# refresh-bio/agc

Hardware: AMD Instinct MI355X
Metric: input Gbp/s compressed (create), hot path FASTA bytes in HBM -> 2-bit pack + scan + match + encode + zstd packing (higher is better)
Workload: dtype u8

## Files before the change

### agc_amd/capi.py

```python
import ctypes as C
import os

import numpy as np

HERE = os.path.dirname(os.path.abspath(__file__))
LIB_PATH = os.path.join(HERE, "libagc_hip.so")

OK, ENODEV, EINVAL, ENOMEM, ECAP, ENOREF = 0, -1, -2, -3, -4, -5
K_SCAN, K_INDEX, K_ENCODE, K_ESTIMATE, K_COSTVEC, K_REVCOMP, K_PREPROCESS, K_REFSTORE = range(8)
K_NAMES = ["scan", "index", "encode", "estimate", "costvec", "revcomp", "preprocess", "refstore", "zstd", "filter", "segments", "pack"]

SYMBOLS = [
    "agc_hip_create", "agc_hip_destroy", "agc_hip_last_error", "agc_hip_abi_version", "agc_hip_sync",
    "agc_hip_timing_enable", "agc_hip_timing_reset", "agc_hip_timing_get",
    "agc_hip_sample_buffer", "agc_hip_copy_to_device",
    "agc_hip_preprocess_dev", "agc_hip_preprocess",
    "agc_hip_splitters_set", "agc_hip_splitters_insert", "agc_hip_splitters_count",
    "agc_hip_determine_splitters_dev",
    "agc_hip_scan_contigs_dev", "agc_hip_scan_contigs",
    "agc_hip_ref_register", "agc_hip_ref_register_batch_dev", "agc_hip_ref_get", "agc_hip_ref_index_get",
    "agc_hip_lz_encode_batch_dev", "agc_hip_lz_encode_batch", "agc_hip_lz_encode_begin_dev", "agc_hip_lz_encode_end", "agc_hip_lz_encode_pending",
    "agc_hip_lz_encode_begin_packed_on", "agc_hip_lz_encode_end_on", "agc_hip_lz_encode_pending_on", "agc_hip_lz_encode_drop_on",
    "agc_hip_host_alloc", "agc_hip_host_free",
    "agc_hip_lz_estimate_batch_dev", "agc_hip_lz_estimate_batch",
    "agc_hip_lz_cost_vector_batch_dev", "agc_hip_lz_cost_vector_batch",
    "agc_hip_lz_split_point_batch_dev", "agc_hip_fetch_slices_dev",
    "agc_hip_ref_lag_counts_dev",
    "agc_hip_zstd17_max_input", "agc_hip_zstd17_resident_frames", "agc_hip_zstd17_batch", "agc_hip_zstd17_batch_dev", "agc_hip_zstd17_background", "agc_hip_zstd17_cparams", "agc_hip_zstd_batch", "agc_hip_zstd_cparams",
    "agc_hip_packed_words_bytes", "agc_hip_packed_index_bytes", "agc_hip_pack_dev", "agc_hip_expand_dev", "agc_hip_scan_packed_dev",
    "agc_hip_prefetch_packed_dev", "agc_hip_scan_prefetched", "agc_hip_sample_pack", "agc_hip_sample_pack_fasta", "agc_hip_ref_store_begin_packed", "agc_hip_ref_store_end",
    "agc_hip_ref_register_batch_packed", "agc_hip_lz_encode_batch_packed", "agc_hip_lz_encode_begin_packed", "agc_hip_lz_estimate_batch_packed",
    "agc_hip_lz_cost_vector_batch_packed", "agc_hip_lz_split_point_batch_packed", "agc_hip_fetch_slices_packed", "agc_hip_ref_lag_counts_packed",
    "agc_hip_pack_fasta_begin", "agc_hip_pack_fasta_end", "agc_hip_pack_fasta_dev",
    "agc_hip_group_hash", "agc_hip_group_map_set", "agc_hip_group_map_update", "agc_hip_segments_packed", "agc_hip_segments_encode_known",
]

u8p = C.POINTER(C.c_uint8)
u32p = C.POINTER(C.c_uint32)
u64p = C.POINTER(C.c_uint64)
vp = C.c_void_p


class Packed(C.Structure):
    _fields_ = [("d_words", C.c_void_p), ("d_esc_index", C.c_void_p), ("d_esc_bytes", C.c_void_p), ("n_symbols", C.c_uint64)]


class GroupSlot(C.Structure):
    _fields_ = [("k1", C.c_uint64), ("k2", C.c_uint64), ("gid", C.c_int32), ("used", C.c_uint32)]


class Segment(C.Structure):
    _fields_ = [("start", C.c_uint64), ("front_dir", C.c_uint64), ("front_rc", C.c_uint64), ("back_dir", C.c_uint64), ("back_rc", C.c_uint64),
                ("ctg", C.c_uint32), ("len", C.c_uint32), ("map_gid", C.c_int32), ("front_full", C.c_uint8), ("back_full", C.c_uint8),
                ("store_rc", C.c_uint8), ("encoded", C.c_uint8)]


# ... 58 lines not shown
    L.agc_hip_lz_estimate_batch_dev.argtypes = [vp, C.c_uint32, u32p, vp, u64p, u32p, u8p, u32p, u32p]
    L.agc_hip_lz_estimate_batch.argtypes = [vp, C.c_uint32, u32p, u8p, u64p, u32p, u8p, u32p, u32p]
    L.agc_hip_lz_cost_vector_batch_dev.argtypes = [vp, C.c_uint32, u32p, vp, u64p, u32p, u8p, u8p, u32p]
    L.agc_hip_lz_cost_vector_batch.argtypes = [vp, C.c_uint32, u32p, u8p, u64p, u32p, u8p, u8p, u32p]
    L.agc_hip_lz_split_point_batch_dev.argtypes = [vp, C.c_uint32, u32p, u32p, vp, u64p, u32p, u8p, u8p, u8p, u8p, u32p, u32p]
    L.agc_hip_fetch_slices_dev.argtypes = [vp, C.c_uint32, vp, u64p, u32p, u8p, u8p, C.c_uint64, u64p]
    L.agc_hip_ref_lag_counts_dev.argtypes = [vp, C.c_uint32, vp, u64p, u32p, u8p, u32p, u32p]
    L.agc_hip_zstd17_batch.argtypes = [vp, C.c_uint32, u8p, u64p, u8p, C.c_uint64, u64p]
    L.agc_hip_zstd17_cparams.argtypes = [C.c_uint64, u32p]
    L.agc_hip_zstd_cparams.argtypes = [C.c_int, C.c_uint64, u32p]
    L.agc_hip_zstd_batch.argtypes = [vp, C.c_uint32, u8p, u64p, u8p, u8p, C.c_uint64, u64p]
    L.agc_hip_zstd17_batch_dev.argtypes = [vp, C.c_uint32, vp, u64p, u8p, C.c_uint64, u64p]
    L.agc_hip_zstd17_background.argtypes = [vp, C.c_int]
    L.agc_hip_zstd17_max_input.restype = C.c_uint32
    L.agc_hip_zstd17_resident_frames.argtypes = [vp]
    L.agc_hip_zstd17_resident_frames.restype = C.c_uint32
    L.agc_hip_packed_words_bytes.restype = C.c_uint64
    L.agc_hip_packed_words_bytes.argtypes = [C.c_uint64]
    L.agc_hip_packed_index_bytes.restype = C.c_uint64
    L.agc_hip_packed_index_bytes.argtypes = [C.c_uint64]
    L.agc_hip_pack_dev.argtypes = [vp, vp, C.c_uint64, vp, vp, vp, C.c_uint64, u64p]
    L.agc_hip_pack_fasta_begin.argtypes = [vp, vp, C.c_uint64, u64p, u64p, C.c_uint32, vp, vp, vp, C.c_uint64]
    L.agc_hip_pack_fasta_end.argtypes = [vp, u64p, u64p]
    L.agc_hip_pack_fasta_dev.argtypes = [vp, vp, C.c_uint64, u64p, u64p, C.c_uint32, vp, vp, vp, C.c_uint64, u64p, u64p]
    L.agc_hip_expand_dev.argtypes = [vp, C.POINTER(Packed), vp]
    L.agc_hip_scan_packed_dev.argtypes = [vp, C.POINTER(Packed), u64p, C.c_uint32, C.c_uint32, C.c_uint64, u64p, u32p, u64p, u64p, u64p]
    L.agc_hip_prefetch_packed_dev.argtypes = [vp, C.POINTER(Packed), u64p, C.c_uint32, C.c_uint32]
    pkp = C.POINTER(Packed)
    L.agc_hip_sample_pack.argtypes = [vp, vp, C.c_uint64, pkp]
    L.agc_hip_ref_store_begin_packed.argtypes = [vp, C.c_uint32, C.c_uint32, C.c_uint32, pkp, u64p, C.POINTER(C.c_uint32), vp, vp, vp, vp, C.c_uint64, u64p]
    L.agc_hip_ref_store_end.argtypes = [vp, C.c_uint32]
    L.agc_hip_sample_pack_fasta.argtypes = [vp, C.c_uint32, C.POINTER(C.c_char_p), u64p, pkp, u64p]
    L.agc_hip_ref_register_batch_packed.argtypes = [vp, C.c_uint32, u32p, pkp, u64p, u32p, u8p, C.c_uint32]
    L.agc_hip_lz_encode_batch_packed.argtypes = [vp, C.c_uint32, u32p, pkp, u64p, u32p, u8p, u8p, C.c_uint64, u64p]
    L.agc_hip_lz_encode_begin_packed.argtypes = [vp, C.c_uint32, u32p, pkp, u64p, u32p, u8p]
    L.agc_hip_lz_encode_begin_packed_on.argtypes = [vp, C.c_uint32, C.c_uint32, u32p, pkp, u64p, u32p, u8p]
    L.agc_hip_lz_encode_end_on.argtypes = [vp, C.c_uint32, u8p, C.c_uint64, u64p]
    L.agc_hip_lz_encode_pending_on.argtypes = [vp, C.c_uint32, u32p]
    L.agc_hip_lz_encode_drop_on.argtypes = [vp, C.c_uint32]
    L.agc_hip_lz_estimate_batch_packed.argtypes = [vp, C.c_uint32, u32p, pkp, u64p, u32p, u8p, u32p, u32p]
    L.agc_hip_lz_cost_vector_batch_packed.argtypes = [vp, C.c_uint32, u32p, pkp, u64p, u32p, u8p, u8p, u32p]
    L.agc_hip_lz_split_point_batch_packed.argtypes = [vp, C.c_uint32, u32p, u32p, pkp, u64p, u32p, u8p, u8p, u8p, u8p, u32p, u32p]
    L.agc_hip_fetch_slices_packed.argtypes = [vp, C.c_uint32, pkp, u64p, u32p, u8p, u8p, C.c_uint64, u64p]
    L.agc_hip_ref_lag_counts_packed.argtypes = [vp, C.c_uint32, pkp, u64p, u32p, u8p, u32p, u32p]
    L.agc_hip_group_hash.argtypes = [C.c_uint64, C.c_uint64]
    L.agc_hip_group_hash.restype = C.c_uint64
# ... 152 lines not shown
        self._chk(self.L.agc_hip_pack_fasta_begin(self.h, d_raw_tensor.data_ptr(), int(n_raw), _p(rb, u64p), _p(re_, u64p), rb.size, words.data_ptr(),
                                                  index.data_ptr(), esc.data_ptr(), esc_cap))
        return {"raw": d_raw_tensor, "n_raw": int(n_raw), "rb": rb, "re": re_, "bufs": (words, index, esc)}

    def pack_fasta_end(self, pending):
        import torch
        while True:
            off = np.zeros(pending["rb"].size + 1, np.uint64)
            cnt = np.zeros(1, np.uint64)
            rc = self.L.agc_hip_pack_fasta_end(self.h, _p(off, u64p), _p(cnt, u64p))
            if rc == ECAP:
                words, index, _esc = pending["bufs"]
                esc = torch.empty((int(cnt[0]) + 16) * 1024, dtype=torch.uint8, device=words.device)
                torch.cuda.synchronize(words.device)
                pending = self.pack_fasta_begin(pending["raw"], pending["n_raw"], pending["rb"], pending["re"], bufs=(words, index, esc))
                continue
            self._chk(rc)
            words, index, esc = pending["bufs"]
            return Packed(words.data_ptr(), index.data_ptr(), esc.data_ptr(), int(off[-1])), pending["bufs"], off

    def pack_fasta_dev(self, d_raw_tensor, n_raw, raw_begin, raw_end, esc_cap=64):
        return self.pack_fasta_end(self.pack_fasta_begin(d_raw_tensor, n_raw, raw_begin, raw_end, esc_cap))

    def expand_dev(self, pk, d_codes_ptr):
        self._chk(self.L.agc_hip_expand_dev(self.h, C.byref(pk), d_codes_ptr))
        self._chk(self.L.agc_hip_sync(self.h))

    def scan_packed_dev(self, pk, ctg_off, k, cap=1 << 16):
        fn = lambda h, arg, *rest: self.L.agc_hip_scan_packed_dev(h, C.byref(arg), *rest)
        return self._scan(fn, pk, ctg_off, k, cap)

    def prefetch_packed_dev(self, pk, ctg_off, k):
        off = _a(ctg_off, np.uint64)
        self._chk(self.L.agc_hip_prefetch_packed_dev(self.h, C.byref(pk), _p(off, u64p), off.size - 1, k))

    def sample_pack(self, d_codes_ptr, n_symbols):
        pk = Packed()
        self._chk(self.L.agc_hip_sample_pack(self.h, d_codes_ptr, n_symbols, C.byref(pk)))
        return pk

    def sample_pack_fasta(self, bodies):
        n = len(bodies)
        ptr = (C.c_char_p * max(n, 1))(*bodies)
        ln = np.array([len(b) for b in bodies], np.uint64)
        off = np.zeros(n + 1, np.uint64)
        pk = Packed()
# ... 287 lines not shown
```

### agc_amd/csrc/api.hip

```cpp
#include "../../include/agc_hip.h"
#include "dev_common.h"

#include <algorithm>
#include <atomic>
#include <chrono>
#include <cstdio>
#include <cstring>
#include <future>
#include <mutex>
#include <numeric>
#include <string>
#include <vector>

#include "scan_kernels.hip"
#include "pack_kernels.hip"
#include "lz_kernels.hip"
#include "seg_kernels.hip"
#include "zstd_kernels.hip"

using namespace agc;

namespace {

struct DevBuf {
// ... 100 lines not shown
        bool done_valid = false;
        hipStream_t s = nullptr;
    } l2, l3;
    hipStream_t stream2 = nullptr, stream3 = nullptr;
    Lane2 &lane(int which) { return which == 2 ? l3 : l2; }

    struct Prefetch {
        hipStream_t stream = nullptr;
        DevBuf d_ranges, d_hits, d_counter;
        uint32_t *h_count = nullptr;
        const void *words = nullptr;
        uint64_t n_symbols = 0;
        uint32_t dev_cap = 0, k = 0, n_ctg = 0;
        uint64_t first_off = 0, last_off = 0;
        bool valid = false, scanned = false;
        hipEvent_t e0 = nullptr, e1 = nullptr;
        bool timed = false;
    } pf;

    struct PackFasta {
        hipStream_t stream = nullptr;
        DevBuf d_state, d_rng, d_off;
        DevBuf d_tcnt, d_toff;
        uint64_t *h_res = nullptr;
        size_t h_res_cap = 0;
        uint32_t n_ctg = 0;
        uint64_t n_raw = 0, esc_cap = 0;
        bool pending = false, timed = false;
        hipEvent_t e0 = nullptr, e1 = nullptr;
    } pfa;

    struct ChunkBufs {
        DevBuf d_jobs, d_seg0, d_logs, d_logn, d_out;
        std::future<DevBuf> logs_ahead;
        bool logs_asked = false;
    } chunk_bufs[3];

    std::vector<void *> host_allocs;

    bool timing = false;
    hipEvent_t ev0 = nullptr, ev1 = nullptr, zev0 = nullptr, zev1 = nullptr;
    struct TimerPair {
        hipEvent_t a = nullptr, b = nullptr;
        int which = -1;
    };
    std::vector<TimerPair> tpairs;
// ... 885 lines not shown
    uint64_t prev = 0;
    for (uint32_t i = 0; i < n_ctg; ++i) {
        if (h_raw_begin[i] < prev || h_raw_end[i] < h_raw_begin[i] || h_raw_end[i] > n_raw)
            return AGC_HIP_EINVAL;
        prev = h_raw_end[i];
    }
    const uint64_t n_tiles64 = (n_raw + PF_TILE - 1) / PF_TILE;
    if (n_tiles64 > 0x7fffffffULL)
        return AGC_HIP_EINVAL;
    HIPCHK(c, hipSetDevice(c->device));
    agc_hip_ctx::PackFasta &P = c->pfa;
    if (!P.stream) {
        HIPCHK(c, hipStreamCreateWithFlags(&P.stream, hipStreamNonBlocking));
        HIPCHK(c, hipEventCreate(&P.e0));
        HIPCHK(c, hipEventCreate(&P.e1));
    }
    if (P.pending) {
        HIPCHK(c, hipStreamSynchronize(P.stream));
        P.pending = false;
    }
    P.n_ctg = n_ctg;
    P.n_raw = n_raw;
    P.esc_cap = esc_cap_blocks;
    const size_t res_words = (size_t)n_ctg + 4;
    if (P.h_res_cap < res_words) {
        if (P.h_res)
            HIPCHK(c, hipHostFree(P.h_res));
        P.h_res = nullptr;
        P.h_res_cap = 0;
        HIPCHK(c, hipHostMalloc((void **)&P.h_res, (res_words + 1024) * 8, hipHostMallocDefault));
        P.h_res_cap = res_words + 1024;
    }
    const uint32_t n_tiles = (uint32_t)n_tiles64;
    CHK(ensure(c, P.d_state, 64, P.stream));
    CHK(ensure(c, P.d_rng, std::max<size_t>(16, (size_t)n_ctg * 16), P.stream));
    CHK(ensure(c, P.d_off, ((size_t)n_ctg + 2) * 8, P.stream));
    HIPCHK(c, hipMemsetAsync(P.d_state.p, 0, 64, P.stream));
    HIPCHK(c, hipMemsetAsync(P.d_off.p, 0xFF, ((size_t)n_ctg + 1) * 8, P.stream));
    if (n_ctg) {
        CHK(upload(c, P.d_rng.p, h_raw_begin, (size_t)n_ctg * 8, P.stream));
        CHK(upload(c, (uint8_t *)P.d_rng.p + (size_t)n_ctg * 8, h_raw_end, (size_t)n_ctg * 8, P.stream));
    }
    P.timed = c->timing;
    if (P.timed)
        (void)hipEventRecord(P.e0, P.stream);
    if (n_tiles && n_ctg) {
        PackFastaArgs a;
        a.raw = d_raw;
        a.n_raw = n_raw;
        a.rng_begin = (const uint64_t *)P.d_rng.p;
        a.rng_end = a.rng_begin + n_ctg;
        a.n_rng = n_ctg;
        a.n_tiles = n_tiles;
        a.esc_count = (uint32_t *)P.d_state.p + 1;
        a.total = (unsigned long long *)P.d_state.p + 1;
        a.words = d_words;
        a.esc_index = d_esc_index;
        a.esc_bytes = d_esc_bytes;
        a.esc_cap = (uint32_t)std::min<uint64_t>(esc_cap_blocks, 0x7fffffffu);
        a.ctg_off = (unsigned long long *)P.d_off.p;
        {
            const uint32_t n_sb = (n_tiles + PF_SCAN_TILES - 1) / PF_SCAN_TILES;
            const size_t tl_bytes = ((size_t)n_tiles * 4 + 255) & ~(size_t)255;
            CHK(ensure(c, P.d_tcnt, tl_bytes + (size_t)n_sb * 4 + 64, P.stream));
            CHK(ensure(c, P.d_toff, tl_bytes + (size_t)n_sb * 8 + 64, P.stream));
            uint32_t *d_cnt = (uint32_t *)P.d_tcnt.p, *d_tot = (uint32_t *)((uint8_t *)P.d_tcnt.p + tl_bytes);
            uint32_t *d_local = (uint32_t *)P.d_toff.p;
            uint64_t *d_boff = (uint64_t *)((uint8_t *)P.d_toff.p + tl_bytes);
            a.tile_local = d_local;
            a.block_off = d_boff;
            hipLaunchKernelGGL(pack_fasta_count_kernel, dim3(n_tiles), dim3(256), 0, P.stream, a, d_cnt);
            hipLaunchKernelGGL(pack_fasta_scan_kernel, dim3(n_sb), dim3(1024), 0, P.stream, (const uint32_t *)d_cnt, n_tiles, d_local, d_tot);
            hipLaunchKernelGGL(pp_scan_kernel, dim3(1), dim3(1024), 0, P.stream, (const uint32_t *)d_tot, n_sb, d_boff,
                               (uint64_t *)((uint8_t *)P.d_state.p + 32));
            hipLaunchKernelGGL(pack_fasta_kernel, dim3(n_tiles), dim3(256), 0, P.stream, a);
        }
        HIPCHK(c, hipGetLastError());
    }
    if (P.timed)
        (void)hipEventRecord(P.e1, P.stream);
    HIPCHK(c, hipMemcpyAsync(P.h_res, P.d_off.p, ((size_t)n_ctg + 1) * 8, hipMemcpyDeviceToHost, P.stream));
    HIPCHK(c, hipMemcpyAsync(P.h_res + n_ctg + 1, P.d_state.p, 16, hipMemcpyDeviceToHost, P.stream));
    P.pending = true;
    return AGC_HIP_OK;
}

int agc_hip_pack_fasta_end(agc_hip_ctx *c, uint64_t *h_ctg_off, uint64_t *h_n_esc_blocks)
{
    if (!c || !h_ctg_off || !h_n_esc_blocks)
        return AGC_HIP_EINVAL;
    agc_hip_ctx::PackFasta &P = c->pfa;
    if (!P.pending)
        return AGC_HIP_EINVAL;
    HIPCHK(c, hipSetDevice(c->device));
    HIPCHK(c, hipStreamSynchronize(P.stream));
    P.pending = false;
    if (P.timed) {
        float ms = 0;
        (void)hipEventElapsedTime(&ms, P.e0, P.e1);
        c->ms[AGC_HIP_K_PACK] += ms;
        c->launches[AGC_HIP_K_PACK] += 1;
        P.timed = false;
    }
    const uint32_t n = P.n_ctg;
    const uint32_t *cnt = (const uint32_t *)(P.h_res + n + 1);
    const uint64_t total = (P.n_raw && n) ? P.h_res[n + 2] : 0;
    for (uint32_t i = 0; i < n; ++i)
        h_ctg_off[i] = P.h_res[i] == ~0ULL ? total : P.h_res[i];
    h_ctg_off[n] = total;
    *h_n_esc_blocks = (P.n_raw && n) ? cnt[1] : 0;
    return *h_n_esc_blocks > P.esc_cap ? AGC_HIP_ECAP : AGC_HIP_OK;
}

int agc_hip_pack_fasta_dev(agc_hip_ctx *c, const uint8_t *d_raw, uint64_t n_raw, const uint64_t *h_raw_begin, const uint64_t *h_raw_end, uint32_t n_ctg,
                           uint32_t *d_words, int32_t *d_esc_index, uint8_t *d_esc_bytes, uint64_t esc_cap_blocks, uint64_t *h_ctg_off, uint64_t *h_n_esc_blocks)
{
    if (!h_ctg_off || !h_n_esc_blocks)
        return AGC_HIP_EINVAL;
    CHK(agc_hip_pack_fasta_begin(c, d_raw, n_raw, h_raw_begin, h_raw_end, n_ctg, d_words, d_esc_index, d_esc_bytes, esc_cap_blocks));
    return agc_hip_pack_fasta_end(c, h_ctg_off, h_n_esc_blocks);
}

int agc_hip_sample_pack_fasta(agc_hip_ctx *c, uint32_t n_ctg, const uint8_t *const *h_raw, const uint64_t *h_len, agc_hip_packed *out, uint64_t *h_ctg_off)
{
    if (!c || !out || !h_ctg_off || (n_ctg && (!h_raw || !h_len)))
        return AGC_HIP_EINVAL;
    *out = agc_hip_packed{};
    HIPCHK(c, hipSetDevice(c->device));
    if (c->pfa.pending) {
        c->err = "sample_pack_fasta: a conversion queued by agc_hip_pack_fasta_begin is pending";
        return AGC_HIP_EINVAL;
    }
    std::vector<uint64_t> rb(n_ctg), re(n_ctg);
    uint64_t tot = 0;
    for (uint32_t i = 0; i < n_ctg; ++i) {
// ... 1744 lines not shown
```

### agc_amd/csrc/pack_kernels.hip

```cpp
#pragma once

namespace agc {

constexpr uint32_t PF_TILE = 16384;
constexpr uint32_t PF_MAX_BLOCKS = PF_TILE / PACK_BLOCK + 1;

struct PackFastaArgs {
    const uint8_t *raw;
    uint64_t n_raw;
    const uint64_t *rng_begin, *rng_end;
    uint32_t n_rng;
    uint32_t n_tiles;
    const uint32_t *tile_local;
    const uint64_t *block_off;
    uint32_t *words;
    int32_t *esc_index;
    uint8_t *esc_bytes;
    uint32_t *esc_count;
    uint32_t esc_cap;
    unsigned long long *ctg_off;
    unsigned long long *total;
};

struct PfChunk {
    uint32_t bits;
    uint32_t cnt;
    uint32_t keep;
    uint32_t other;
};

__device__ __forceinline__ uint8_t pf_byte(const uint32_t w[4], uint32_t j)
{
    const uint32_t q = j >> 2, x = q == 0 ? w[0] : q == 1 ? w[1] : q == 2 ? w[2] : w[3];
    return (uint8_t)(x >> (8 * (j & 3)));
}

__device__ __forceinline__ uint32_t pf_ge64(uint32_t w) { return ((w << 1) | w) & 0x80808080u; }

__device__ __forceinline__ uint32_t pf_gather16(uint32_t f0, uint32_t f1, uint32_t f2, uint32_t f3)
{
    uint32_t v = (f0 >> 7) | (f1 >> 6) | (f2 >> 5) | (f3 >> 4);
    v = (v | (v >> 4)) & 0x00FF00FFu;
    v = (v | (v >> 8)) & 0xFFFFu;
    uint32_t t = ((v >> 3) ^ v) & 0x0A0Au;
// ... 131 lines not shown
            lds_flag[li / PACK_BLOCK] = 1;
        if (first < 16 && (other >> first))
            lds_flag[li / PACK_BLOCK + 1] = 1;
    }
}

__device__ __forceinline__ void pf_escape(const PackFastaArgs &a, const int32_t *lds_slot, uint64_t g, uint32_t keep, const uint32_t w[4], uint64_t s0, uint64_t s1)
{
    for (uint32_t m = keep; m; m &= m - 1, ++g) {
        if (g < s0 || g >= s1)
            continue;
        const int32_t slot = lds_slot[(g - s0) / PACK_BLOCK];
        if (slot >= 0)
            a.esc_bytes[(uint64_t)slot * PACK_BLOCK + ((g - s0) & (PACK_BLOCK - 1))] = cnv_symbol(pf_byte(w, __builtin_ctz(m)));
    }
}

__global__ void __launch_bounds__(256) pack_fasta_count_kernel(PackFastaArgs a, uint32_t *__restrict__ tile_cnt)
{
    __shared__ uint32_t s_part[4], s_rfirst;
    __shared__ unsigned long long s_cb, s_ce;
    const uint32_t tid = threadIdx.x, lane = tid & 63, wv = tid >> 6, tile = blockIdx.x;
    const uint64_t t_begin = (uint64_t)tile * PF_TILE;
    if (tid == 0) {
        uint32_t lo = 0, hi = a.n_rng;
        while (lo < hi) {
            const uint32_t mid = (lo + hi) >> 1;
            if (a.rng_end[mid] <= t_begin)
                lo = mid + 1;
            else
                hi = mid;
        }
        s_rfirst = lo;
        s_cb = lo < a.n_rng ? a.rng_begin[lo] : ~0ULL;
        s_ce = lo < a.n_rng ? a.rng_end[lo] : 0;
    }
    __syncthreads();
    const uint32_t r_first = s_rfirst;
    const uint64_t cb = s_cb, ce = s_ce;
    uint32_t c = 0;
#pragma unroll
    for (uint32_t j = 0; j < 4; ++j) {
        const uint64_t p = t_begin + (uint64_t)wv * 4096 + j * 1024 + lane * 16;
        if (p >= a.n_raw)
            continue;
        uint32_t w[4] = {0, 0, 0, 0};
// ... 4 lines not shown
#pragma unroll
            for (uint32_t t = 0; t < 16; ++t)
                if (p + t < a.n_raw)
                    w[t >> 2] |= (uint32_t)a.raw[p + t] << (8 * (t & 3));
        }
        const uint32_t m0 = pf_ge64(w[0]), m1 = pf_ge64(w[1]), m2 = pf_ge64(w[2]), m3 = pf_ge64(w[3]);
        if (p >= cb && p + 16 <= ce)
            c += __popc(m0) + __popc(m1) + __popc(m2) + __popc(m3);
        else
            c += __popc(pf_gather16(m0, m1, m2, m3) & pf_range_mask(a, p, cb, ce, r_first));
    }
#pragma unroll
    for (int o = 32; o > 0; o >>= 1)
        c += __shfl_down(c, o);
    if (lane == 0)
        s_part[wv] = c;
    __syncthreads();
    if (tid == 0)
        tile_cnt[tile] = s_part[0] + s_part[1] + s_part[2] + s_part[3];
}

constexpr uint32_t PF_SCAN_TILES = 8192;
__global__ void __launch_bounds__(1024) pack_fasta_scan_kernel(const uint32_t *__restrict__ tile_cnt, uint32_t n_tiles, uint32_t *__restrict__ tile_local,
                                                              uint32_t *__restrict__ block_total)
{
    __shared__ uint32_t s_w[16];
    const uint32_t tid = threadIdx.x, lane = tid & 63, wv = tid >> 6;
    const uint32_t t0 = blockIdx.x * PF_SCAN_TILES + tid * 8;
    uint32_t v[8], sum = 0;
#pragma unroll
    for (uint32_t j = 0; j < 8; ++j) {
        v[j] = t0 + j < n_tiles ? tile_cnt[t0 + j] : 0u;
        sum += v[j];
    }
    const uint32_t incl = pf_wave_incl(sum);
    if (lane == 63)
        s_w[wv] = incl;
    __syncthreads();
    uint32_t base = 0, total = 0;
#pragma unroll
    for (uint32_t x = 0; x < 16; ++x) {
        if (x < wv)
            base += s_w[x];
        total += s_w[x];
    }
    uint32_t run = base + incl - sum;
#pragma unroll
    for (uint32_t j = 0; j < 8; ++j) {
        if (t0 + j < n_tiles)
            tile_local[t0 + j] = run;
        run += v[j];
    }
    if (tid == 0)
        block_total[blockIdx.x] = total;
}

__global__ void __launch_bounds__(256) pack_fasta_kernel(PackFastaArgs a)
{
    __shared__ uint32_t s_words[PF_MAX_BLOCKS * (PACK_BLOCK / 16)];
    __shared__ uint32_t s_flag[PF_MAX_BLOCKS];
    __shared__ int32_t s_slot[PF_MAX_BLOCKS];
    __shared__ uint32_t s_wsum[4 * 4];
    __shared__ uint32_t s_tile, s_rfirst;
    __shared__ unsigned long long s_excl, s_cb, s_ce;
    __shared__ uint32_t s_ra[4];
    const uint32_t tid = threadIdx.x, lane = tid & 63, wv = tid >> 6;

    if (tid == 0)
        s_tile = blockIdx.x;
    for (uint32_t i = tid; i < PF_MAX_BLOCKS * (PACK_BLOCK / 16); i += 256)
        s_words[i] = 0;
    if (tid < PF_MAX_BLOCKS) {
        s_flag[tid] = 0;
        s_slot[tid] = -1;
    }
    __syncthreads();
    const uint32_t tile = s_tile;
    if (tile >= a.n_tiles)
        return;
    const uint64_t t_begin = (uint64_t)tile * PF_TILE, t_end = t_begin + PF_TILE < a.n_raw ? t_begin + PF_TILE : a.n_raw;
    if (tid == 0) {
        uint32_t lo = 0, hi = a.n_rng;
        while (lo < hi) {
            const uint32_t mid = (lo + hi) >> 1;
            if (a.rng_end[mid] <= t_begin)
                lo = mid + 1;
            else
                hi = mid;
        }
        s_rfirst = lo;
// ... 109 lines not shown
    p_next = t_begin + PF_TILE;
    for (uint32_t r = 0; r < n_rounds; ++r) {
        uint32_t wr[4];
        const uint32_t need = (uint32_t)(s1 - g_next), span = min(4096u, (need + need / 16 + 47) & ~15u);
        const PfChunk c = pf_chunk(a, tid * 16 < span ? p_next + tid * 16 : a.n_raw, cb, ce, r_first, wr);
        const uint32_t incl = pf_wave_incl(c.cnt);
        __syncthreads();
        if (lane == 63)
            s_ra[wv] = incl;
        __syncthreads();
        uint32_t base = 0, tot = 0;
#pragma unroll
        for (uint32_t x = 0; x < 4; ++x) {
            if (x < wv)
                base += s_ra[x];
            tot += s_ra[x];
        }
        pf_escape(a, s_slot, g_next + base + incl - c.cnt, c.keep, wr, s0, s1);
        g_next += tot;
        p_next += span;
    }
}

}
```

### agc_amd/csrc/scan_kernels.hip

```cpp
#include "dev_common.h"

namespace agc {

__device__ __forceinline__ uint32_t pack4(uint32_t w)
{
    return ((w & 0x03030303u) * 0x40100401u) >> 24;
}

__device__ __forceinline__ uint32_t inv4(uint32_t w)
{
    uint32_t v = w & 0xFCFCFCFCu;
    uint32_t nz = ((v & 0x7F7F7F7Fu) + 0x7F7F7F7Fu) | v;
    nz &= 0x80808080u;
    return ((nz >> 7) & 1u) << 3 | ((nz >> 15) & 1u) << 2 | ((nz >> 23) & 1u) << 1 | (nz >> 31);
}

__device__ __forceinline__ uint64_t rev2(uint64_t x)
{
    x = __brevll(x);
    return ((x & 0x5555555555555555ULL) << 1) | ((x >> 1) & 0x5555555555555555ULL);
}

struct ScanArgs {
    const uint8_t *codes;
// ... 488 lines not shown
        if (p + 16 <= n) {
            uint4 v;
            __builtin_memcpy(&v, raw + p, 16);
            c += __popc(((v.x >> 6) | (v.x >> 7)) & 0x01010101u);
            c += __popc(((v.y >> 6) | (v.y >> 7)) & 0x01010101u);
            c += __popc(((v.z >> 6) | (v.z >> 7)) & 0x01010101u);
            c += __popc(((v.w >> 6) | (v.w >> 7)) & 0x01010101u);
        } else {
            for (uint32_t j = 0; j < 16 && p + j < n; ++j)
                c += (raw[p + j] >> 6) != 0;
        }
    }
    for (int o = 32; o > 0; o >>= 1)
        c += __shfl_down(c, o);
    __shared__ uint32_t part[4];
    if ((threadIdx.x & 63) == 0)
        part[threadIdx.x >> 6] = c;
    __syncthreads();
    if (threadIdx.x == 0)
        block_cnt[blockIdx.x] = part[0] + part[1] + part[2] + part[3];
}

__global__ void __launch_bounds__(1024) pp_scan_kernel(const uint32_t *__restrict__ block_cnt, uint32_t n_blocks,
                                                       uint64_t *__restrict__ block_off, uint64_t *__restrict__ total)
{
    __shared__ uint64_t s_part[1024];
    const uint32_t per = (n_blocks + blockDim.x - 1) / blockDim.x;
    const uint32_t b = threadIdx.x * per, e = min(b + per, n_blocks);
    uint64_t sum = 0;
    for (uint32_t i = b; i < e; ++i)
        sum += block_cnt[i];
    s_part[threadIdx.x] = sum;
    __syncthreads();
    if (threadIdx.x == 0) {
        uint64_t acc = 0;
        for (uint32_t i = 0; i < blockDim.x; ++i) {
            const uint64_t v = s_part[i];
            s_part[i] = acc;
            acc += v;
        }
        *total = acc;
    }
    __syncthreads();
    uint64_t acc = s_part[threadIdx.x];
    for (uint32_t i = b; i < e; ++i) {
        block_off[i] = acc;
        acc += block_cnt[i];
    }
}
// ... 38 lines not shown
```

### include/agc_hip.h

```cpp
#ifndef AGC_HIP_H
#define AGC_HIP_H

#include <stddef.h>
#include <stdint.h>

#ifdef __cplusplus
extern "C" {
#endif

#define AGC_HIP_OK 0
#define AGC_HIP_ENODEV (-1)
#define AGC_HIP_EINVAL (-2)
#define AGC_HIP_ENOMEM (-3)
#define AGC_HIP_ECAP (-4)
#define AGC_HIP_ENOREF (-5)

typedef struct agc_hip_ctx agc_hip_ctx;

int agc_hip_create(agc_hip_ctx **out, int device);
void agc_hip_destroy(agc_hip_ctx *ctx);
const char *agc_hip_last_error(const agc_hip_ctx *ctx);
uint32_t agc_hip_abi_version(void);
int agc_hip_sync(agc_hip_ctx *ctx);

// ... 37 lines not shown
                             const uint64_t *h_ctg_off, uint32_t n_ctg, uint32_t k,
                             uint64_t cap, uint64_t *h_n_hits,
                             uint32_t *h_hit_ctg, uint64_t *h_hit_pos,
                             uint64_t *h_hit_dir, uint64_t *h_hit_rc);
int agc_hip_scan_contigs(agc_hip_ctx *ctx, const uint8_t *h_codes,
                         const uint64_t *h_ctg_off, uint32_t n_ctg, uint32_t k,
                         uint64_t cap, uint64_t *h_n_hits,
                         uint32_t *h_hit_ctg, uint64_t *h_hit_pos,
                         uint64_t *h_hit_dir, uint64_t *h_hit_rc);

typedef struct {
    const uint32_t *d_words;
    const int32_t *d_esc_index;
    const uint8_t *d_esc_bytes;
    uint64_t n_symbols;
} agc_hip_packed;
uint64_t agc_hip_packed_words_bytes(uint64_t n_symbols);
uint64_t agc_hip_packed_index_bytes(uint64_t n_symbols);
int agc_hip_pack_dev(agc_hip_ctx *ctx, const uint8_t *d_codes, uint64_t n_symbols, uint32_t *d_words, int32_t *d_esc_index,
                     uint8_t *d_esc_bytes, uint64_t esc_cap_blocks, uint64_t *h_n_esc_blocks);
int agc_hip_pack_fasta_begin(agc_hip_ctx *ctx, const uint8_t *d_raw, uint64_t n_raw, const uint64_t *h_raw_begin, const uint64_t *h_raw_end,
                             uint32_t n_ctg, uint32_t *d_words, int32_t *d_esc_index, uint8_t *d_esc_bytes, uint64_t esc_cap_blocks);
int agc_hip_pack_fasta_end(agc_hip_ctx *ctx, uint64_t *h_ctg_off, uint64_t *h_n_esc_blocks);
int agc_hip_pack_fasta_dev(agc_hip_ctx *ctx, const uint8_t *d_raw, uint64_t n_raw, const uint64_t *h_raw_begin, const uint64_t *h_raw_end,
                           uint32_t n_ctg, uint32_t *d_words, int32_t *d_esc_index, uint8_t *d_esc_bytes, uint64_t esc_cap_blocks,
                           uint64_t *h_ctg_off, uint64_t *h_n_esc_blocks);
int agc_hip_sample_pack_fasta(agc_hip_ctx *ctx, uint32_t n_ctg, const uint8_t *const *h_raw, const uint64_t *h_len, agc_hip_packed *out,
                              uint64_t *h_ctg_off);
int agc_hip_expand_dev(agc_hip_ctx *ctx, const agc_hip_packed *pk, uint8_t *d_codes);
int agc_hip_sample_pack(agc_hip_ctx *ctx, const uint8_t *d_codes, uint64_t n_symbols, agc_hip_packed *out);
int agc_hip_scan_packed_dev(agc_hip_ctx *ctx, const agc_hip_packed *pk, const uint64_t *h_ctg_off, uint32_t n_ctg, uint32_t k,
                            uint64_t cap, uint64_t *h_n_hits, uint32_t *h_hit_ctg, uint64_t *h_hit_pos,
                            uint64_t *h_hit_dir, uint64_t *h_hit_rc);
int agc_hip_prefetch_packed_dev(agc_hip_ctx *ctx, const agc_hip_packed *pk, const uint64_t *h_ctg_off, uint32_t n_ctg, uint32_t k);
int agc_hip_scan_prefetched(agc_hip_ctx *ctx, const agc_hip_packed *pk, const uint64_t *h_ctg_off, uint32_t n_ctg, uint32_t k,
                            uint64_t cap, uint64_t *h_n_hits, uint32_t *h_hit_ctg, uint64_t *h_hit_pos, uint64_t *h_hit_dir,
                            uint64_t *h_hit_rc);

typedef struct {
    uint64_t k1, k2;
    int32_t gid;
    uint32_t used;
} agc_hip_group_slot;
uint64_t agc_hip_group_hash(uint64_t k1, uint64_t k2);
int agc_hip_group_map_set(agc_hip_ctx *ctx, const agc_hip_group_slot *h_slots, uint64_t n_slots);
int agc_hip_group_map_update(agc_hip_ctx *ctx, uint32_t n, const uint64_t *h_idx, const agc_hip_group_slot *h_slots);
// ... 132 lines not shown
```

Before: 37.08.

## Add fixed-line-width FASTA fast path computing symbol positions arithmetically

```diff
diff --git a/agc_amd/capi.py b/agc_amd/capi.py
--- a/agc_amd/capi.py
+++ b/agc_amd/capi.py
@@ -9,6 +9,8 @@
 OK, ENODEV, EINVAL, ENOMEM, ECAP, ENOREF = 0, -1, -2, -3, -4, -5
 K_SCAN, K_INDEX, K_ENCODE, K_ESTIMATE, K_COSTVEC, K_REVCOMP, K_PREPROCESS, K_REFSTORE = range(8)
 K_NAMES = ["scan", "index", "encode", "estimate", "costvec", "revcomp", "preprocess", "refstore", "zstd", "filter", "segments", "pack"]
+
+PACK_PATH_NONE, PACK_PATH_REGULAR, PACK_PATH_GENERAL = 0, 1, 2
 
 SYMBOLS = [
     "agc_hip_create", "agc_hip_destroy", "agc_hip_last_error", "agc_hip_abi_version", "agc_hip_sync",
@@ -31,7 +33,7 @@
     "agc_hip_prefetch_packed_dev", "agc_hip_scan_prefetched", "agc_hip_sample_pack", "agc_hip_sample_pack_fasta", "agc_hip_ref_store_begin_packed", "agc_hip_ref_store_end",
     "agc_hip_ref_register_batch_packed", "agc_hip_lz_encode_batch_packed", "agc_hip_lz_encode_begin_packed", "agc_hip_lz_estimate_batch_packed",
     "agc_hip_lz_cost_vector_batch_packed", "agc_hip_lz_split_point_batch_packed", "agc_hip_fetch_slices_packed", "agc_hip_ref_lag_counts_packed",
-    "agc_hip_pack_fasta_begin", "agc_hip_pack_fasta_end", "agc_hip_pack_fasta_dev",
+    "agc_hip_pack_fasta_begin", "agc_hip_pack_fasta_end", "agc_hip_pack_fasta_dev", "agc_hip_pack_fasta_path",
     "agc_hip_group_hash", "agc_hip_group_map_set", "agc_hip_group_map_update", "agc_hip_segments_packed", "agc_hip_segments_encode_known",
 ]
 
@@ -136,6 +138,7 @@
     L.agc_hip_pack_dev.argtypes = [vp, vp, C.c_uint64, vp, vp, vp, C.c_uint64, u64p]
     L.agc_hip_pack_fasta_begin.argtypes = [vp, vp, C.c_uint64, u64p, u64p, C.c_uint32, vp, vp, vp, C.c_uint64]
     L.agc_hip_pack_fasta_end.argtypes = [vp, u64p, u64p]
+    L.agc_hip_pack_fasta_path.argtypes = [vp]
     L.agc_hip_pack_fasta_dev.argtypes = [vp, vp, C.c_uint64, u64p, u64p, C.c_uint32, vp, vp, vp, C.c_uint64, u64p, u64p]
     L.agc_hip_expand_dev.argtypes = [vp, C.POINTER(Packed), vp]
     L.agc_hip_scan_packed_dev.argtypes = [vp, C.POINTER(Packed), u64p, C.c_uint32, C.c_uint32, C.c_uint64, u64p, u32p, u64p, u64p, u64p]
@@ -334,6 +337,9 @@
     def pack_fasta_dev(self, d_raw_tensor, n_raw, raw_begin, raw_end, esc_cap=64):
         return self.pack_fasta_end(self.pack_fasta_begin(d_raw_tensor, n_raw, raw_begin, raw_end, esc_cap))
 
+    def pack_fasta_path(self):
+        return int(self.L.agc_hip_pack_fasta_path(self.h))
+
     def expand_dev(self, pk, d_codes_ptr):
         self._chk(self.L.agc_hip_expand_dev(self.h, C.byref(pk), d_codes_ptr))
         self._chk(self.L.agc_hip_sync(self.h))
diff --git a/agc_amd/csrc/api.hip b/agc_amd/csrc/api.hip
--- a/agc_amd/csrc/api.hip
+++ b/agc_amd/csrc/api.hip
@@ -146,6 +146,9 @@
         hipStream_t stream = nullptr;
         DevBuf d_state, d_rng, d_off;
         DevBuf d_tcnt, d_toff;
+        DevBuf d_shape, d_nsym, d_soff;
+        bool regular = false;
+        int path = 0;
         uint64_t *h_res = nullptr;
         size_t h_res_cap = 0;
         uint32_t n_ctg = 0;
@@ -1077,7 +1080,7 @@
     P.n_ctg = n_ctg;
     P.n_raw = n_raw;
     P.esc_cap = esc_cap_blocks;
-    const size_t res_words = (size_t)n_ctg + 4;
+    const size_t res_words = 2 * ((size_t)n_ctg + 1) + 8;
     if (P.h_res_cap < res_words) {
         if (P.h_res)
             HIPCHK(c, hipHostFree(P.h_res));
@@ -1087,10 +1090,14 @@
         P.h_res_cap = res_words + 1024;
     }
     const uint32_t n_tiles = (uint32_t)n_tiles64;
+    const char *sw = getenv("AGC_HIP_PACK_REGULAR");
+    P.regular = !(sw && atoi(sw) == 0) && n_tiles64 && n_ctg;
     CHK(ensure(c, P.d_state, 64, P.stream));
     CHK(ensure(c, P.d_rng, std::max<size_t>(16, (size_t)n_ctg * 16), P.stream));
     CHK(ensure(c, P.d_off, ((size_t)n_ctg + 2) * 8, P.stream));
     HIPCHK(c, hipMemsetAsync(P.d_state.p, 0, 64, P.stream));
+    if (!P.regular)
+        HIPCHK(c, hipMemsetAsync(P.d_state.p, 1, 4, P.stream));
     HIPCHK(c, hipMemsetAsync(P.d_off.p, 0xFF, ((size_t)n_ctg + 1) * 8, P.stream));
     if (n_ctg) {
         CHK(upload(c, P.d_rng.p, h_raw_begin, (size_t)n_ctg * 8, P.stream));
@@ -1114,6 +1121,30 @@
         a.esc_bytes = d_esc_bytes;
         a.esc_cap = (uint32_t)std::min<uint64_t>(esc_cap_blocks, 0x7fffffffu);
         a.ctg_off = (unsigned long long *)P.d_off.p;
+        a.irregular = (const uint32_t *)P.d_state.p;
+        if (P.regular) {
+            CHK(ensure(c, P.d_shape, (size_t)n_ctg * 8, P.stream));
+            CHK(ensure(c, P.d_nsym, (size_t)n_ctg * 8, P.stream));
+            CHK(ensure(c, P.d_soff, ((size_t)n_ctg + 1) * 8, P.stream));
+            PackRegArgs r;
+            r.raw = d_raw;
+            r.n_raw = n_raw;
+            r.rng_begin = a.rng_begin;
+            r.rng_end = a.rng_end;
+            r.n_rng = n_ctg;
+            r.shape = (uint2 *)P.d_shape.p;
+            r.n_sym = (unsigned long long *)P.d_nsym.p;
+            r.sym_off = (unsigned long long *)P.d_soff.p;
+            r.words = d_words;
+            r.esc_index = d_esc_index;
+            r.esc_bytes = d_esc_bytes;
+            r.esc_count = (uint32_t *)P.d_state.p + 4;
+            r.esc_cap = a.esc_cap;
+            r.irregular = (uint32_t *)P.d_state.p;
+            hipLaunchKernelGGL(pack_shape_kernel, dim3(n_ctg), dim3(64), 0, P.stream, r);
+            hipLaunchKernelGGL(pack_shape_scan_kernel, dim3(1), dim3(1024), 0, P.stream, r);
+            hipLaunchKernelGGL(pack_regular_kernel, dim3((uint32_t)((n_raw + PR_WG_SYMS - 1) / PR_WG_SYMS)), dim3(256), 0, P.stream, r);
+        }
         {
             const uint32_t n_sb = (n_tiles + PF_SCAN_TILES - 1) / PF_SCAN_TILES;
             const size_t tl_bytes = ((size_t)n_tiles * 4 + 255) & ~(size_t)255;
@@ -1125,9 +1156,9 @@
             a.tile_local = d_local;
             a.block_off = d_boff;
             hipLaunchKernelGGL(pack_fasta_count_kernel, dim3(n_tiles), dim3(256), 0, P.stream, a, d_cnt);
-            hipLaunchKernelGGL(pack_fasta_scan_kernel, dim3(n_sb), dim3(1024), 0, P.stream, (const uint32_t *)d_cnt, n_tiles, d_local, d_tot);
+            hipLaunchKernelGGL(pack_fasta_scan_kernel, dim3(n_sb), dim3(1024), 0, P.stream, (const uint32_t *)d_cnt, n_tiles, d_local, d_tot, a.irregular);
             hipLaunchKernelGGL(pp_scan_kernel, dim3(1), dim3(1024), 0, P.stream, (const uint32_t *)d_tot, n_sb, d_boff,
-                               (uint64_t *)((uint8_t *)P.d_state.p + 32));
+                               (uint64_t *)((uint8_t *)P.d_state.p + 32), a.irregular);
             hipLaunchKernelGGL(pack_fasta_kernel, dim3(n_tiles), dim3(256), 0, P.stream, a);
         }
         HIPCHK(c, hipGetLastError());
@@ -1135,7 +1166,9 @@
     if (P.timed)
         (void)hipEventRecord(P.e1, P.stream);
     HIPCHK(c, hipMemcpyAsync(P.h_res, P.d_off.p, ((size_t)n_ctg + 1) * 8, hipMemcpyDeviceToHost, P.stream));
-    HIPCHK(c, hipMemcpyAsync(P.h_res + n_ctg + 1, P.d_state.p, 16, hipMemcpyDeviceToHost, P.stream));
+    HIPCHK(c, hipMemcpyAsync(P.h_res + n_ctg + 1, P.d_state.p, 32, hipMemcpyDeviceToHost, P.stream));
+    if (P.regular)
+        HIPCHK(c, hipMemcpyAsync(P.h_res + n_ctg + 5, P.d_soff.p, ((size_t)n_ctg + 1) * 8, hipMemcpyDeviceToHost, P.stream));
     P.pending = true;
     return AGC_HIP_OK;
 }
@@ -1159,6 +1192,17 @@
     }
     const uint32_t n = P.n_ctg;
     const uint32_t *cnt = (const uint32_t *)(P.h_res + n + 1);
+    P.path = !(P.n_raw && n) ? AGC_HIP_PACK_PATH_NONE : (P.regular && !cnt[0]) ? AGC_HIP_PACK_PATH_REGULAR : AGC_HIP_PACK_PATH_GENERAL;
+    static const bool laps = getenv("AGC_HIP_LAPS") != nullptr;
+    if (laps)
+        fprintf(stderr, "    pack_fasta: %s path, %.1f MB of FASTA, %u contigs\n",
+                P.path == AGC_HIP_PACK_PATH_REGULAR ? "regular" : P.path == AGC_HIP_PACK_PATH_GENERAL ? "general" : "no", P.n_raw / 1e6, n);
+    if (P.path == AGC_HIP_PACK_PATH_REGULAR) {
+        for (uint32_t i = 0; i <= n; ++i)
+            h_ctg_off[i] = P.h_res[n + 5 + i];
+        *h_n_esc_blocks = cnt[4];
+        return *h_n_esc_blocks > P.esc_cap ? AGC_HIP_ECAP : AGC_HIP_OK;
+    }
     const uint64_t total = (P.n_raw && n) ? P.h_res[n + 2] : 0;
     for (uint32_t i = 0; i < n; ++i)
         h_ctg_off[i] = P.h_res[i] == ~0ULL ? total : P.h_res[i];
@@ -1166,6 +1210,8 @@
     *h_n_esc_blocks = (P.n_raw && n) ? cnt[1] : 0;
     return *h_n_esc_blocks > P.esc_cap ? AGC_HIP_ECAP : AGC_HIP_OK;
 }
+
+int agc_hip_pack_fasta_path(agc_hip_ctx *c) { return c ? c->pfa.path : AGC_HIP_EINVAL; }
 
 int agc_hip_pack_fasta_dev(agc_hip_ctx *c, const uint8_t *d_raw, uint64_t n_raw, const uint64_t *h_raw_begin, const uint64_t *h_raw_end, uint32_t n_ctg,
                            uint32_t *d_words, int32_t *d_esc_index, uint8_t *d_esc_bytes, uint64_t esc_cap_blocks, uint64_t *h_ctg_off, uint64_t *h_n_esc_blocks)
diff --git a/agc_amd/csrc/pack_kernels.hip b/agc_amd/csrc/pack_kernels.hip
--- a/agc_amd/csrc/pack_kernels.hip
+++ b/agc_amd/csrc/pack_kernels.hip
@@ -20,6 +20,7 @@
     uint32_t esc_cap;
     unsigned long long *ctg_off;
     unsigned long long *total;
+    const uint32_t *irregular;
 };
 
 struct PfChunk {
@@ -197,6 +198,8 @@
     __shared__ unsigned long long s_cb, s_ce;
     const uint32_t tid = threadIdx.x, lane = tid & 63, wv = tid >> 6, tile = blockIdx.x;
     const uint64_t t_begin = (uint64_t)tile * PF_TILE;
+    if (!*a.irregular)
+        return;
     if (tid == 0) {
         uint32_t lo = 0, hi = a.n_rng;
         while (lo < hi) {
@@ -247,9 +250,11 @@
 
 constexpr uint32_t PF_SCAN_TILES = 8192;
 __global__ void __launch_bounds__(1024) pack_fasta_scan_kernel(const uint32_t *__restrict__ tile_cnt, uint32_t n_tiles, uint32_t *__restrict__ tile_local,
-                                                              uint32_t *__restrict__ block_total)
+                                                              uint32_t *__restrict__ block_total, const uint32_t *__restrict__ irregular)
 {
     __shared__ uint32_t s_w[16];
+    if (!*irregular)
+        return;
     const uint32_t tid = threadIdx.x, lane = tid & 63, wv = tid >> 6;
     const uint32_t t0 = blockIdx.x * PF_SCAN_TILES + tid * 8;
     uint32_t v[8], sum = 0;
@@ -291,6 +296,8 @@
     __shared__ uint32_t s_ra[4];
     const uint32_t tid = threadIdx.x, lane = tid & 63, wv = tid >> 6;
 
+    if (!*a.irregular)
+        return;
     if (tid == 0)
         s_tile = blockIdx.x;
     for (uint32_t i = tid; i < PF_MAX_BLOCKS * (PACK_BLOCK / 16); i += 256)
@@ -446,4 +453,364 @@
     }
 }
 
-}
+constexpr uint32_t PR_WG_BLOCKS = 16;
+constexpr uint32_t PR_WG_SYMS = PR_WG_BLOCKS * PACK_BLOCK;
+constexpr uint32_t PR_MAX_LINE = 1u << 20;
+
+struct PackRegArgs {
+    const uint8_t *raw;
+    uint64_t n_raw;
+    const uint64_t *rng_begin, *rng_end;
+    uint32_t n_rng;
+    uint2 *shape;
+    unsigned long long *n_sym;
+    unsigned long long *sym_off;
+    uint32_t *words;
+    int32_t *esc_index;
+    uint8_t *esc_bytes;
+    uint32_t *esc_count;
+    uint32_t esc_cap;
+    uint32_t *irregular;
+};
+
+__global__ void __launch_bounds__(64) pack_shape_kernel(PackRegArgs a)
+{
+    const uint32_t c = blockIdx.x, lane = threadIdx.x;
+    const uint64_t b = a.rng_begin[c], e = a.rng_end[c], len = e - b;
+    const uint64_t lim = len < PR_MAX_LINE ? e : b + PR_MAX_LINE;
+    uint64_t first = ~0ULL;
+    for (uint64_t p0 = b & ~15ULL; p0 < lim; p0 += 1024) {
+        const uint64_t p = p0 + lane * 16;
+        uint32_t w[4] = {0x40404040u, 0x40404040u, 0x40404040u, 0x40404040u};
+        if (p < lim) {
+            if (p + 16 <= a.n_raw) {
+                const uint4 v = *(const uint4 *)(a.raw + p);
+                w[0] = v.x, w[1] = v.y, w[2] = v.z, w[3] = v.w;
+            } else {
+#pragma unroll
+                for (uint32_t t = 0; t < 16; ++t)
+                    if (p + t < a.n_raw)
+                        w[t >> 2] = (w[t >> 2] & ~(0xFFu << (8 * (t & 3)))) | ((uint32_t)a.raw[p + t] << (8 * (t & 3)));
+            }
+        }
+        uint32_t low = ~pf_gather16(pf_ge64(w[0]), pf_ge64(w[1]), pf_ge64(w[2]), pf_ge64(w[3])) & 0xFFFFu;
+        if (p < b)
+            low &= b - p >= 16 ? 0u : 0xFFFFu << (uint32_t)(b - p);
+        if (p + 16 > lim)
+            low &= p >= lim ? 0u : 0xFFFFu >> (uint32_t)(p + 16 - lim);
+        const uint64_t hit = __ballot(low != 0);
+        if (hit) {
+            const uint32_t src = (uint32_t)__builtin_ctzll(hit);
+            const uint32_t m = (uint32_t)__shfl((int)low, (int)src);
+            first = p0 + src * 16 + __builtin_ctz(m);
+            break;
+        }
+    }
+    if (lane)
+        return;
+    uint32_t L = 0, E = 0;
+    uint64_t n = 0;
+    bool ok = true;
+    if (first == ~0ULL) {
+        ok = len <= PR_MAX_LINE;
+        L = (uint32_t)(ok ? len : 0);
+        n = L;
+    } else {
+        L = (uint32_t)(first - b);
+        E = 1;
+        if (first + 1 < e && a.raw[first + 1] < 64) {
+            E = 2;
+            if (first + 2 < e && a.raw[first + 2] < 64)
+                ok = false;
+        }
+        if (L == 0)
+            ok = false;
+        if (ok) {
+            uint32_t T = 0;
+            if (a.raw[e - 1] < 64) {
+                T = 1;
+                if (E == 2 && len >= 2 && a.raw[e - 2] < 64)
+                    T = 2;
+            }
+            const uint64_t body = len - T, S = (uint64_t)L + E, q = body / S, r = body % S;
+            if (r == 0 || r > L)
+                ok = false;
+            else
+                n = q * L + r;
+        }
+    }
+    if (!ok) {
+        L = E = 0;
+        n = 0;
+        *a.irregular = 1;
+    }
+    a.shape[c] = make_uint2(L, E);
+    a.n_sym[c] = n;
+}
+
+__global__ void __launch_bounds__(1024) pack_shape_scan_kernel(PackRegArgs a)
+{
+    __shared__ unsigned long long s_part[1024];
+    const uint32_t per = (a.n_rng + blockDim.x - 1) / blockDim.x;
+    const uint32_t b = min(threadIdx.x * per, a.n_rng), e = min(b + per, a.n_rng);
+    unsigned long long sum = 0;
+    for (uint32_t i = b; i < e; ++i)
+        sum += a.n_sym[i];
+    s_part[threadIdx.x] = sum;
+    __syncthreads();
+    if (threadIdx.x == 0) {
+        unsigned long long acc = 0;
+        for (uint32_t i = 0; i < blockDim.x; ++i) {
+            const unsigned long long v = s_part[i];
+            s_part[i] = acc;
+            acc += v;
+        }
+        a.sym_off[a.n_rng] = acc;
+    }
+    __syncthreads();
+    unsigned long long acc = s_part[threadIdx.x];
+    for (uint32_t i = b; i < e; ++i) {
+        a.sym_off[i] = acc;
+        acc += a.n_sym[i];
+    }
+}
+
+struct PrLoc {
+    uint32_t c, L, E, rem;
+    uint64_t begin, end, n, i;
+    uint64_t pos;
+};
+
+struct PrHome {
+    uint32_t c, L, E, r0;
+    float inv_l;
+    uint64_t begin, end, off, n, line0, g0;
+};
+
+__device__ __forceinline__ PrLoc pr_locate(const PackRegArgs &a, const PrHome &h, uint64_t g)
+{
+    PrLoc l;
+    uint64_t line;
+    if (g < h.off + h.n) {
+        l.c = h.c, l.L = h.L, l.E = h.E, l.begin = h.begin, l.end = h.end, l.n = h.n;
+        l.i = g - h.off;
+        const uint32_t x = h.r0 + (uint32_t)(g - h.g0);
+        uint32_t q = (uint32_t)((float)x * h.inv_l);
+        int32_t r = (int32_t)(x - q * h.L);
+        if (r < 0)
+            --q, r += (int32_t)h.L;
+        else if ((uint32_t)r >= h.L)
+            ++q, r -= (int32_t)h.L;
+        l.rem = (uint32_t)r;
+        line = h.line0 + q;
+    } else {
+        uint32_t lo = h.c + 1, hi = a.n_rng - 1;
+        while (lo < hi) {
+            const uint32_t mid = (lo + hi) >> 1;
+            if (a.sym_off[mid + 1] <= g)
+                lo = mid + 1;
+            else
+                hi = mid;
+        }
+        const uint2 sh = a.shape[lo];
+        l.c = lo, l.L = sh.x, l.E = sh.y, l.begin = a.rng_begin[lo], l.end = a.rng_end[lo];
+        const uint64_t off = a.sym_off[lo];
+        l.n = a.sym_off[lo + 1] - off;
+        l.i = g - off;
+        const uint32_t x = (uint32_t)l.i;
+        line = x / l.L;
+        l.rem = x % l.L;
+    }
+    l.pos = l.begin + l.i + line * l.E;
+    return l;
+}
+
+__device__ __forceinline__ void pr_next_contig(const PackRegArgs &a, PrLoc &l)
+{
+    do {
+        ++l.c;
+        l.n = a.sym_off[l.c + 1] - a.sym_off[l.c];
+    } while (!l.n);
+    const uint2 sh = a.shape[l.c];
+    l.L = sh.x, l.E = sh.y, l.begin = a.rng_begin[l.c], l.end = a.rng_end[l.c];
+    l.i = 0, l.rem = 0, l.pos = l.begin;
+}
+
+__device__ __forceinline__ uint32_t pr_prefix(uint32_t k, uint32_t q)
+{
+    const int32_t nb = (int32_t)k - (int32_t)(4 * q);
+    return nb >= 4 ? 0xFFFFFFFFu : nb <= 0 ? 0u : (1u << (8 * nb)) - 1u;
+}
+
+__device__ __forceinline__ uint32_t pr_word(const PackRegArgs &a, const PrHome &h, uint64_t g, uint64_t total, bool &other, bool &bad)
+{
+    PrLoc l = pr_locate(a, h, g);
+    const uint32_t k = l.L - l.rem;
+    const uint64_t base = l.pos & ~3ULL;
+    if (l.i + 16 < l.n && (uint64_t)k + l.L > 16 && base + 24 <= a.n_raw) {
+        struct __attribute__((aligned(4))) Q { uint32_t x, y, z, w; };
+        struct __attribute__((aligned(4))) D { uint32_t x, y; };
+        const Q d0 = *(const Q *)(a.raw + base);
+        const D d1 = *(const D *)(a.raw + base + 16);
+        const uint32_t sh = (uint32_t)l.pos & 3u;
+        uint32_t A[5], w[4];
+        A[0] = __builtin_amdgcn_alignbyte(d0.y, d0.x, sh);
+        A[1] = __builtin_amdgcn_alignbyte(d0.z, d0.y, sh);
+        A[2] = __builtin_amdgcn_alignbyte(d0.w, d0.z, sh);
+        A[3] = __builtin_amdgcn_alignbyte(d1.x, d0.w, sh);
+        A[4] = __builtin_amdgcn_alignbyte(d1.y, d1.x, sh);
+        if (k < 16) {
+#pragma unroll
+            for (uint32_t q = 0; q < 4; ++q) {
+                const uint32_t B = __builtin_amdgcn_alignbyte(A[q + 1], A[q], l.E), m = pr_prefix(k, q);
+                w[q] = (A[q] & m) | (B & ~m);
+            }
+        } else {
+#pragma unroll
+            for (uint32_t q = 0; q < 4; ++q)
+                w[q] = A[q];
+        }
+        uint32_t all = 0x80808080u, odd = 0, diffs[4], code[4];
+#pragma unroll
+        for (uint32_t q = 0; q < 4; ++q) {
+            const uint32_t x = w[q];
+            all &= pf_ge64(x);
+            const uint32_t t = (x >> 1) & 0x03030303u;
+            code[q] = __builtin_amdgcn_perm(0u, 0x02030100u, t);
+            const uint32_t expect = __builtin_amdgcn_perm(0u, 0x47544341u, t);
+            diffs[q] = (x & 0xDFDFDFDFu) ^ expect;
+            odd |= diffs[q];
+        }
+        if (all != 0x80808080u)
+            bad = true;
+        if (k <= 16) {
+            const uint32_t tail = l.E == 1 ? 0x80u : 0x8080u;
+            const uint32_t low = __popc(~pf_ge64(A[0]) & 0x80808080u) + __popc(~pf_ge64(A[1]) & 0x80808080u) + __popc(~pf_ge64(A[2]) & 0x80808080u) +
+                                 __popc(~pf_ge64(A[3]) & 0x80808080u) + __popc(~pf_ge64(A[4]) & tail);
+            if (low != l.E)
+                bad = true;
+        }
+        uint32_t u = code[0] | (code[1] << 2) | (code[2] << 4) | (code[3] << 6);
+        uint32_t t = ((u >> 6) ^ u) & 0x00CC00CCu;
+        u ^= t ^ (t << 6);
+        t = ((u >> 12) ^ u) & 0x0000F0F0u;
+        u ^= t ^ (t << 12);
+        if (odd) {
+            other = true;
+#pragma unroll
+            for (uint32_t q = 0; q < 4; ++q)
+                for (uint32_t j = 0; j < 4; ++j)
+                    if ((diffs[q] >> (8 * j)) & 0xFFu) {
+                        const uint32_t f = 2 * (4 * q + j);
+                        u = (u & ~(3u << f)) | ((uint32_t)(cnv_symbol((uint8_t)(w[q] >> (8 * j))) & 3u) << f);
+                    }
+        }
+        return u;
+    }
+    uint32_t u = 0;
+    for (uint32_t j = 0; j < 16 && g + j < total; ++j) {
+        if (l.i == l.n)
+            pr_next_contig(a, l);
+        const uint8_t x = a.raw[l.pos];
+        if (x < 64)
+            bad = true;
+        const uint32_t code = cnv_symbol(x);
+        other |= code > 3;
+        u |= (code & 3u) << (2 * j);
+        const bool last = l.i + 1 == l.n, eol = l.rem + 1 == l.L;
+        const uint64_t n_end = last ? l.end - l.pos - 1 : eol ? l.E : 0;
+        if (n_end > l.E)
+            bad = true;
+        for (uint32_t t = 0; t < n_end && t < 2; ++t)
+            if (a.raw[l.pos + 1 + t] >= 64)
+                bad = true;
+        ++l.i;
+        ++l.pos;
+        if (eol)
+            l.rem = 0, l.pos += l.E;
+        else
+            ++l.rem;
+    }
+    return u;
+}
+
+__global__ void __launch_bounds__(256) pack_regular_kernel(PackRegArgs a)
+{
+    __shared__ uint32_t s_flag[PR_WG_BLOCKS];
+    __shared__ int32_t s_slot[PR_WG_BLOCKS];
+    __shared__ PrHome s_home;
+    __shared__ uint32_t s_skip;
+    const uint32_t tid = threadIdx.x;
+    const uint64_t total = a.sym_off[a.n_rng], g0 = (uint64_t)blockIdx.x * PR_WG_SYMS;
+    if (g0 >= total)
+        return;
+    if (tid < PR_WG_BLOCKS)
+        s_flag[tid] = 0;
+    if (tid == 0) {
+        s_skip = *(volatile uint32_t *)a.irregular;
+        uint32_t lo = 0, hi = a.n_rng - 1;
+        while (lo < hi) {
+            const uint32_t mid = (lo + hi) >> 1;
+            if (a.sym_off[mid + 1] <= g0)
+                lo = mid + 1;
+            else
+                hi = mid;
+        }
+        PrHome h;
+        const uint2 sh = a.shape[lo];
+        h.c = lo, h.L = sh.x, h.E = sh.y, h.begin = a.rng_begin[lo], h.end = a.rng_end[lo], h.off = a.sym_off[lo];
+        h.n = a.sym_off[lo + 1] - h.off;
+        h.g0 = g0;
+        const uint64_t i0 = g0 - h.off;
+        h.line0 = i0 / h.L;
+        h.r0 = (uint32_t)(i0 % h.L);
+        h.inv_l = 1.0f / (float)h.L;
+        s_home = h;
+    }
+    __syncthreads();
+    if (s_skip)
+        return;
+    const PrHome h = s_home;
+    const uint32_t n_own = (uint32_t)min((uint64_t)PR_WG_BLOCKS, (total - g0 + PACK_BLOCK - 1) / PACK_BLOCK);
+    bool bad = false;
+#pragma unroll 1
+    for (uint32_t j = 0; j < PR_WG_SYMS / 16 / 256; ++j) {
+        const uint32_t wi = j * 256 + tid;
+        if (wi >= n_own * (PACK_BLOCK / 16))
+            break;
+        const uint64_t g = g0 + (uint64_t)wi * 16;
+        uint32_t u = 0;
+        if (g < total) {
+            bool other = false;
+            u = pr_word(a, h, g, total, other, bad);
+            if (other)
+                s_flag[wi / (PACK_BLOCK / 16)] = 1;
+        }
+        a.words[g / 16] = u;
+    }
+    if (bad)
+        *a.irregular = 1;
+    __syncthreads();
+    if (tid < n_own) {
+        int32_t slot = -1;
+        if (s_flag[tid]) {
+            const uint32_t s = atomicAdd(a.esc_count, 1u);
+            slot = s < a.esc_cap ? (int32_t)s : -2;
+        }
+        s_slot[tid] = slot;
+        a.esc_index[g0 / PACK_BLOCK + tid] = slot;
+    }
+    __syncthreads();
+    for (uint32_t b = 0; b < n_own; ++b) {
+        const int32_t slot = s_slot[b];
+        if (slot < 0)
+            continue;
+        for (uint32_t s = tid; s < PACK_BLOCK; s += 256) {
+            const uint64_t g = g0 + (uint64_t)b * PACK_BLOCK + s;
+            if (g < total)
+                a.esc_bytes[(uint64_t)slot * PACK_BLOCK + s] = cnv_symbol(a.raw[pr_locate(a, h, g).pos]);
+        }
+    }
+}
+
+}
diff --git a/agc_amd/csrc/scan_kernels.hip b/agc_amd/csrc/scan_kernels.hip
--- a/agc_amd/csrc/scan_kernels.hip
+++ b/agc_amd/csrc/scan_kernels.hip
@@ -534,9 +534,12 @@
 }
 
 __global__ void __launch_bounds__(1024) pp_scan_kernel(const uint32_t *__restrict__ block_cnt, uint32_t n_blocks,
-                                                       uint64_t *__restrict__ block_off, uint64_t *__restrict__ total)
+                                                       uint64_t *__restrict__ block_off, uint64_t *__restrict__ total,
+                                                       const uint32_t *__restrict__ only_if = nullptr)
 {
     __shared__ uint64_t s_part[1024];
+    if (only_if && !*only_if)
+        return;
     const uint32_t per = (n_blocks + blockDim.x - 1) / blockDim.x;
     const uint32_t b = threadIdx.x * per, e = min(b + per, n_blocks);
     uint64_t sum = 0;
diff --git a/include/agc_hip.h b/include/agc_hip.h
--- a/include/agc_hip.h
+++ b/include/agc_hip.h
@@ -83,6 +83,8 @@
 int agc_hip_pack_fasta_begin(agc_hip_ctx *ctx, const uint8_t *d_raw, uint64_t n_raw, const uint64_t *h_raw_begin, const uint64_t *h_raw_end,
                              uint32_t n_ctg, uint32_t *d_words, int32_t *d_esc_index, uint8_t *d_esc_bytes, uint64_t esc_cap_blocks);
 int agc_hip_pack_fasta_end(agc_hip_ctx *ctx, uint64_t *h_ctg_off, uint64_t *h_n_esc_blocks);
+enum { AGC_HIP_PACK_PATH_NONE = 0, AGC_HIP_PACK_PATH_REGULAR = 1, AGC_HIP_PACK_PATH_GENERAL = 2 };
+int agc_hip_pack_fasta_path(agc_hip_ctx *ctx);
 int agc_hip_pack_fasta_dev(agc_hip_ctx *ctx, const uint8_t *d_raw, uint64_t n_raw, const uint64_t *h_raw_begin, const uint64_t *h_raw_end,
                            uint32_t n_ctg, uint32_t *d_words, int32_t *d_esc_index, uint8_t *d_esc_bytes, uint64_t esc_cap_blocks,
                            uint64_t *h_ctg_off, uint64_t *h_n_esc_blocks);
```

New measurement: 27.76. -25.1%, worse.
